# sortmerna/sortmerna

Hardware: AMD Instinct MI355X
Metric: reads/sec (150 bp vs smr_v4.3_default_db-sized DB) (higher is better)
Workload: dtype u8/i32

## Files before the change

### sortmerna_amd/csrc/smr_engine.hip

```cpp
#include <hip/hip_runtime.h>

#include <algorithm>
#include <mutex>
#include <cstdio>
#include <cstdlib>
#include <cstring>
#include <string>
#include <vector>

#include "smr_kernels.hpp"
#include "smr_idcov.hpp"
#include "smr_ibuild.hpp"
#include "smr_pgbuild.hpp"
#include "smr_hostmem.hpp"

using namespace smr;

namespace {

struct DevIndex {
  bool used = false;
  Lookup* lookup = nullptr; uint32_t* trie = nullptr; uint32_t* pos_off = nullptr; uint2* pos_arr = nullptr;
  uint32_t* pg = nullptr; uint32_t* root3 = nullptr; uint32_t* lkc = nullptr;
  uint8_t* ref_seq = nullptr; uint64_t* ref_off = nullptr;
// ... 8 lines not shown

#define SMR_MAX_BATCHES 16
enum { KP_KEYS = 0, KP_SPLIT, KP_BINS, KP_PG0, KP_PG1, KP_FINISH, KP_CAND, KP_CHAIN, KP_BEGINS, KP_TRACE, KP_WALK, KP_SW16, KP_WNEXT, KP_IDCOV, KP_COUNT };
static const char* const KP_NAME[KP_COUNT] = {"k_seed_keys", "k_seed_split", "k_seed_bins", "k_seed_pg<0>", "k_seed_pg<1>", "k_seed_finish", "k_cand", "k_chain", "k_begins", "k_trace",
                                              "k_walk", "k_sw16", "k_wnext", "k_idcov"};

struct Batch {
  bool used = false;
  uint32_t n = 0, max_len = 0, slots = 1;
  uint32_t min_ge[7] = {~0u, ~0u, ~0u, ~0u, ~0u, ~0u, ~0u};
  uint64_t gen = 0;
  bool min_ge_known = false;
  uint32_t* d_words = nullptr; uint64_t* d_rec_off = nullptr; uint32_t* d_len = nullptr;
  RState* d_saved = nullptr; RState* d_work = nullptr; RWork* d_rw = nullptr;
  uint8_t* d_marks = nullptr;
  AlignRec* d_saved_aln = nullptr; AlignRec* d_work_aln = nullptr;
  unsigned long long* d_ctr = nullptr;
  uint32_t* d_cigar = nullptr; uint64_t cigar_words = 0;
  uint32_t* d_idcov = nullptr; size_t cap_idcov = 0; bool idcov_ran = false;
  std::vector<uint32_t> h_idcov;
  std::vector<RState> h_state; std::vector<AlignRec> h_aln; std::vector<uint32_t> h_cigar;
  std::vector<uint32_t> h_idx, h_map;
  uint32_t last_num_alignments = 1;
  unsigned long long redo_seen = 0, win_seen = 0;
  bool fetched = false;
  size_t cap_words = 0, cap_reads = 0, cap_aln = 0;
};

struct SharedSet { SeedTup* srt = nullptr; uint16_t* wbin = nullptr; uint32_t* cbase = nullptr; uint32_t* sn = nullptr; uint32_t maxwin = 0; bool built = false; };
struct SharedSort {
  SharedSet set[2][3];
  const void* batch = nullptr; uint64_t gen = 0; uint32_t lnwin = 0, skip[3] = {0, 0, 0}, n = 0, max_len = 0;
  uint64_t cap[3] = {0, 0, 0};
  bool usable = false;
  uint32_t* abits = nullptr; size_t abits_words = 0;
};

struct smr_ctx {
  int device = 0;
  hipStream_t stream = nullptr;
  std::string err;
  std::mutex err_m, sel_m;
  int n_cu = 256;
  DevIndex idx[64];
  Batch bt[SMR_MAX_BATCHES];
  Batch* b = &bt[0];
  uint32_t* d_pool = nullptr; uint64_t pool_words = 0;
  uint64_t n_pool_grown = 0;
  uint32_t pool_inline = 0;
  uint32_t hcap = 4;
  int seed_exact = 0;
  uint32_t cand_bloom = 128;
  uint32_t hot_min = getenv("SMR_SEED_DEDUP") ? (uint32_t)std::max(0, atoi(getenv("SMR_SEED_DEDUP"))) : 1024u;
  int seed_shared = getenv("SMR_SEED_SHARED") ? atoi(getenv("SMR_SEED_SHARED")) : 1;
  uint16_t* d_sw_scr = nullptr; uint32_t sw_scr_stride = 0; size_t sw_scr_words = 0;
  int last_seed_slot = -1;
  SharedSort* shared = nullptr;
  uint64_t n_seed_shared = 0, n_seed_shared_builds = 0;
  uint32_t ccap = PG_CAND_CAP0;
  uint32_t pg_grid = getenv("SMR_PG_GRID") ? (uint32_t)atoi(getenv("SMR_PG_GRID")) : 262144u;
  int pg_swz = getenv("SMR_PG_SWZ") ? atoi(getenv("SMR_PG_SWZ")) : 0;
  SeedBufs sb = {};
  uint64_t sb_slots = 0; uint32_t sb_nk = 0;
  uint32_t chain_blocks = 0;
  unsigned long long* d_tuples = nullptr; uint32_t chain_scap = 512;
  uint32_t keys_need = 0;
  bool chain_ext = false;
  uint32_t* d_stab = nullptr; unsigned long long* d_tuples2 = nullptr;
  size_t chain_lds_attr = 0, begins_lds_attr = 0, split_lds_attr = 0, bins_lds_attr = 0;
  uint32_t* d_fidx = nullptr; RState* d_fstate = nullptr; AlignRec* d_faln = nullptr; size_t fetch_cap_r = 0, fetch_cap_a = 0;
  uint32_t* d_fidcov = nullptr; size_t fetch_cap_i = 0;
  int sw_mode = getenv("SMR_SW_PACKED") ? atoi(getenv("SMR_SW_PACKED")) : 2;
  unsigned long long* d_keys = nullptr; uint32_t keys_cap = 0;
  unsigned long long* d_pairs = nullptr; uint32_t* d_lis = nullptr; uint32_t pairs_cap = 0;
  uint2* d_hits = nullptr; uint32_t hits_cap = 0;
  uint8_t* d_rdq = nullptr; size_t rdq_cap = 0;
  int handover = getenv("SMR_HANDOVER") ? atoi(getenv("SMR_HANDOVER")) : 1;
  uint2* d_mrec = nullptr; uint32_t* d_mpool = nullptr; size_t mrec_cap = 0, mpool_words = 0;
  int walk_split = getenv("SMR_WALK_SPLIT") ? atoi(getenv("SMR_WALK_SPLIT")) : 1;
  uint32_t walk_rounds = getenv("SMR_WALK_ROUNDS") ? (uint32_t)std::max(1, std::min(32, atoi(getenv("SMR_WALK_ROUNDS")))) : 8u;
  uint32_t walk_k = getenv("SMR_WALK_K") ? (uint32_t)std::max(1, std::min((int)WK_MAX, atoi(getenv("SMR_WALK_K")))) : 4u;
  int walk_gather = getenv("SMR_WALK_GATHER") ? atoi(getenv("SMR_WALK_GATHER")) : 1;
  uint32_t walk_assume = getenv("SMR_WALK_ASSUME") ? (uint32_t)atoi(getenv("SMR_WALK_ASSUME")) : 3u;
  uint2* d_wlist[2] = {nullptr, nullptr}; WState* d_wstate[2] = {nullptr, nullptr}; WTask* d_wtask[2] = {nullptr, nullptr}; uint2* d_wres[2] = {nullptr, nullptr};
  uint32_t* d_wtidx = nullptr; uint32_t* d_wslow = nullptr; unsigned long long* d_wctr = nullptr; size_t walk_cap = 0; uint32_t walk_kcap = 0, walk_rcap = 0;
  size_t walk_lds_attr = 0, pg_lds_attr = 0, search_lds_attr = 0;
  uint64_t sw16_launches[8] = {};
  bool walk_rounds_fixed = getenv("SMR_WALK_ROUNDS") != nullptr;
  uint32_t walk_need[3] = {0, 0, 0};
  unsigned long long* d_wstat = nullptr; uint32_t wstat_n = 0; int wstat_pass[8] = {}; uint32_t wstat_rm[8] = {};
  int* d_bound = nullptr; size_t bound_cap = 0;
  uint32_t* d_tasks = nullptr; uint64_t tasks_cap = 0;
  uint8_t* d_trflags = nullptr; uint64_t trflags_bytes = 0;
  int* d_trrows = nullptr; uint64_t trrows_ints = 0;
  std::vector<EvMark> events; std::vector<hipEvent_t> ev_pool;
  double kp_ms[KP_COUNT] = {}; uint64_t kp_l[KP_COUNT] = {};
  hipStream_t upload_stream = nullptr;
  unsigned long long* d_ctr_snap = nullptr;
};
struct KpSave { double ms[KP_COUNT]; uint64_t l[KP_COUNT]; };

#define SEED_REDO_CAP 16384u

namespace {

#define HIPCHK(ctx, call)                                                                        \
  do {                                                                                           \
    hipError_t e_ = (call);                                                                      \
    if (e_ != hipSuccess) {                                                                      \
      std::lock_guard<std::mutex> l_((ctx)->err_m);                                              \
      (ctx)->err = std::string(#call) + ": " + hipGetErrorString(e_);                            \
      return SMR_ERR_DEVICE;                                                                     \
    }                                                                                            \
  } while (0)

void set_err(smr_ctx* c, const std::string& msg) { std::lock_guard<std::mutex> l_(c->err_m); c->err = msg; }

template <class T> int dev_alloc(smr_ctx* c, T** p, size_t count) {
  if (*p) { (void)hipFree(*p); *p = nullptr; }
  if (count == 0) count = 1;
  HIPCHK(c, hipMalloc((void**)p, count * sizeof(T)));
  return SMR_OK;
}
template <class T> void dev_free(T** p) { if (*p) { (void)hipFree(*p); *p = nullptr; } }


const char* scheme_unsupported(int mismatch, int score_N, int gap_open, int gap_ext);
DParams make_dparams(const smr_ctx* c, const DevIndex& di, const smr_params* p) {
  DParams P;
  memset(&P, 0, sizeof P);
  P.lnwin = di.lnwin; P.partialwin = di.lnwin / 2;
  if (p->skiplengths[0] == 0 || p->skiplengths[1] == 0 || p->skiplengths[2] == 0) {
    P.skip[0] = di.lnwin; P.skip[1] = di.lnwin / 2; P.skip[2] = 3;
  } else { P.skip[0] = p->skiplengths[0]; P.skip[1] = p->skiplengths[1]; P.skip[2] = p->skiplengths[2]; }
  P.num_seeds = p->num_seeds; P.min_lis = p->min_lis; P.edges = p->edges; P.is_as_percent = p->is_as_percent;
  P.match = p->match; P.mismatch = p->mismatch; P.score_N = p->score_N; P.gap_open = p->gap_open; P.gap_ext = p->gap_ext;
  P.minimal_score = p->minimal_score; P.num_alignments = p->num_alignments;
  P.is_best = p->is_best; P.is_full_search = p->is_full_search; P.is_forward = p->is_forward; P.is_reverse = p->is_reverse;
  P.minoccur = p->minoccur; P.index_num = p->index_num; P.part = p->part; P.is_last_index_part = p->is_last_index_part;
  P.slots = c->b->slots;
  P.sw_mode = scheme_unsupported(p->mismatch, p->score_N, p->gap_open, p->gap_ext) ? -1 : c->sw_mode;
  P.sw_scratch = c->d_sw_scr; P.sw_scratch_stride = c->sw_scr_stride;
  return P;
}

const char* scheme_unsupported(int mismatch, int score_N, int gap_open, int gap_ext) {
  const int mm = std::max(-mismatch, -std::min(score_N, 0));
  if (2 * gap_open < mm || 2 * gap_ext < mm) return "scoring scheme outside the supported range (2*gap_open and 2*gap_ext must be >= |mismatch|)";
  if (score_N > 0) return "scoring scheme outside the supported range (score_N must be <= 0: the kernels pad sequences with N)";
  if (gap_open <= gap_ext) return "scoring scheme outside the supported range (gap_open must be greater than gap_ext: the reference's 16-bit kernel ends its lazy-F loop early otherwise, ssw.c:496-507)";
  return nullptr;
}

int check_params(smr_ctx* c, const smr_params* p, bool sw = true) {
  if (!p) { set_err(c, "null params"); return SMR_ERR_ARG; }
  if (p->index_num >= 64) { set_err(c, "index_num must be < 64"); return SMR_ERR_ARG; }
  if ((uint64_t)p->minoccur >= 0x3FFFFFFFull) { set_err(c, "minoccur must be < 2^30 - 1"); return SMR_ERR_ARG; }
  if (p->num_seeds < 1 || p->gap_open < 0 || p->gap_ext < 0 || p->match <= 0 || p->mismatch > 0) { set_err(c, "bad scoring/seed options"); return SMR_ERR_ARG; }
  if (p->match > 127 || p->mismatch < -127 || p->score_N > 127 || p->score_N < -127 || p->gap_open > 255 || p->gap_ext > 255) { set_err(c, "scores must fit int8 / gaps uint8 like the reference's"); return SMR_ERR_ARG; }
  if (sw && (p->edges < 1 || p->edges > 10)) { set_err(c, "edges must be 1..10 (nucleotides or percent), like the reference's --edges"); return SMR_ERR_ARG; }
  if (p->num_alignments > 0 && p->num_alignments > c->b->slots) { set_err(c, "num_alignments exceeds max_alignments_per_read given to smr_reads_upload"); return SMR_ERR_ARG; }
  return SMR_OK;
}

DIndex dindex(const DevIndex& d) {
  DIndex x; x.lookup = d.lookup; x.trie = d.trie; x.pg = d.pg; x.lkc = d.lkc; x.root3 = reinterpret_cast<const uint2*>(d.root3); x.pos_off = d.pos_off; x.pos_arr = d.pos_arr; x.ref_seq = d.ref_seq; x.ref_off = d.ref_off;
// ... 852 lines not shown
```

### sortmerna_amd/csrc/smr_engine_chain.hpp

```cpp

uint32_t chain_edges(const DParams& P, uint32_t len) { return P.is_as_percent ? (uint32_t)((P.edges / 100.0) * len) + 1 : (uint32_t)std::max(P.edges, 0); }
void chain_lds(const smr_ctx* c, const DParams& P, uint32_t& ml, uint32_t& rf, uint32_t& rq, size_t& bytes) {
  const uint32_t mq_len = std::min<uint32_t>(c->b->max_len, SW_X4_MAX_ROWS);
  ml = (c->b->max_len + 15) & ~15u;
  rf = (c->b->max_len + 2 * chain_edges(P, c->b->max_len) + 16 + 15) & ~15u;
  rq = std::min(rf, (mq_len + 2 * chain_edges(P, mq_len) + 16 + 15) & ~15u);
  bytes = 5 * (size_t)std::min<uint32_t>(ml, SW_X4_MAX_ROWS) + (size_t)9 * rq + (size_t)CH_KEYS_LDS * 8 + (size_t)std::max<uint32_t>(4u * CH_PAIRS_LDS, 2u * c->chain_scap) * 4 +
          (size_t)CH_HITS_LDS * 8 + (size_t)(CH_HITS_LDS + 8) * 4 + (size_t)c->chain_scap * 4;
}
void chain_lds(const smr_ctx* c, const DParams& P, uint32_t& ml, uint32_t& rf, size_t& bytes) { uint32_t rq; chain_lds(c, P, ml, rf, rq, bytes); }
int ensure_bound(smr_ctx* c, uint32_t blocks, uint32_t rf) {
  if (c->b->max_len <= SW_X4_MAX_ROWS) return SMR_OK;
  const size_t need = (size_t)blocks * 2 * rf, need_rd = (size_t)blocks * ((c->b->max_len + 15) & ~15u);
  if (c->bound_cap < need) { int rc = dev_alloc(c, &c->d_bound, need); if (rc) return rc; c->bound_cap = need; }
  if (c->rdq_cap < need_rd) { int rc = dev_alloc(c, &c->d_rdq, need_rd); if (rc) return rc; c->rdq_cap = need_rd; }
  return SMR_OK;
}

__global__ void k_wstat(const unsigned long long* __restrict__ wctr, unsigned long long* __restrict__ out, uint32_t rounds) {
  if (threadIdx.x < 32) out[threadIdx.x] = threadIdx.x < rounds ? wctr[(size_t)threadIdx.x * WC_STRIDE + WC_NLIST] : 0ull;
}
int adapt_walk_rounds(smr_ctx* c) {
  if (c->walk_rounds_fixed || !c->wstat_n || !c->d_wstat) return SMR_OK;
  unsigned long long h[8 * 32];
  HIPCHK(c, hipMemcpyAsync(h, c->d_wstat, (size_t)c->wstat_n * 32 * 8, hipMemcpyDeviceToHost, c->stream));
  HIPCHK(c, hipStreamSynchronize(c->stream));
  const unsigned long long few = (unsigned long long)c->n_cu * 8ull;
  uint32_t need[3] = {0, 0, 0};
  for (uint32_t e = 0; e < c->wstat_n; e++) {
    uint32_t want = 2;
    for (uint32_t r = 0; r < c->wstat_rm[e]; r++) if (h[e * 32 + r] > few) want = r + 2 + (r + 1 == c->wstat_rm[e] ? 2u : 0u);
    need[c->wstat_pass[e]] = std::max(need[c->wstat_pass[e]], want);
  }
  for (int p = 0; p < 3; p++) if (need[p]) {
    const uint32_t prev = c->walk_need[p] ? c->walk_need[p] : c->walk_rounds;
    c->walk_need[p] = std::min(c->walk_rounds, need[p] >= prev ? need[p] : prev - std::max(1u, (prev - need[p]) / 2u));
  }
  c->wstat_n = 0;
  return SMR_OK;
}

int launch_chain(smr_ctx* c, const DevIndex& di, const DParams& P, int pass, int is_last_strand) {
  uint32_t ml, rf, rq; size_t lds;
  chain_lds(c, P, ml, rf, rq, lds);
  HIPCHK(c, hipMemsetAsync(&c->b->d_ctr[C_WORK_NEXT], 0, 8, c->stream));
  if (lds > 64 * 1024 && lds > c->chain_lds_attr) {
    HIPCHK(c, hipFuncSetAttribute((const void*)k_chain<false, false>, hipFuncAttributeMaxDynamicSharedMemorySize, (int)lds));
    HIPCHK(c, hipFuncSetAttribute((const void*)k_chain<true, false>, hipFuncAttributeMaxDynamicSharedMemorySize, (int)lds));
    HIPCHK(c, hipFuncSetAttribute((const void*)k_chain<false, true>, hipFuncAttributeMaxDynamicSharedMemorySize, (int)lds));
    HIPCHK(c, hipFuncSetAttribute((const void*)k_chain<true, true>, hipFuncAttributeMaxDynamicSharedMemorySize, (int)lds));
    HIPCHK(c, hipFuncSetAttribute((const void*)k_chain<false, false, true>, hipFuncAttributeMaxDynamicSharedMemorySize, (int)lds));
    HIPCHK(c, hipFuncSetAttribute((const void*)k_chain<true, false, true>, hipFuncAttributeMaxDynamicSharedMemorySize, (int)lds));
    HIPCHK(c, hipFuncSetAttribute((const void*)k_chain<false, true, true>, hipFuncAttributeMaxDynamicSharedMemorySize, (int)lds));
    HIPCHK(c, hipFuncSetAttribute((const void*)k_chain<true, true, true>, hipFuncAttributeMaxDynamicSharedMemorySize, (int)lds));
    c->chain_lds_attr = lds;
  }
  uint32_t blocks = std::min<uint32_t>(c->chain_blocks, std::max(c->b->n, 1u));
  { int rc = ensure_bound(c, c->chain_blocks, rf); if (rc) return rc; }
  int* const gb = c->b->max_len > SW_X4_MAX_ROWS ? c->d_bound : nullptr;
  uint8_t* const grd = c->b->max_len > SW_X4_MAX_ROWS ? c->d_rdq : nullptr;
  if (c->handover) {
    const size_t want_w = (size_t)((c->b->n + CAND_BLOCK - 1u) / CAND_BLOCK) * CAND_BLOCK * CAND_REC_WORDS;
    if (c->mrec_cap < c->b->n) { int rc = dev_alloc(c, &c->d_mrec, (size_t)c->b->n); if (rc) return rc; c->mrec_cap = c->b->n; }
    if (c->mpool_words < want_w) { int rc = dev_alloc(c, &c->d_mpool, want_w); if (rc) return rc; c->mpool_words = want_w; }
  }
  uint2* const mrec = c->handover ? c->d_mrec : nullptr;
  const uint32_t wmq = std::min<uint32_t>(c->b->max_len, WK_MAX_ROWS), wml = (wmq + 15) & ~15u;
  const bool split = c->walk_split && mrec && P.sw_mode >= 1 && sw_pk_fits((int)wmq, (int)rq, P.match, P.mismatch, P.score_N, P.gap_open);
  const uint32_t RMX = c->walk_rounds, WK = c->walk_k;
  const uint32_t RM = (!c->walk_rounds_fixed && c->walk_need[pass]) ? std::min(RMX, c->walk_need[pass]) : RMX;
  if (split) {
    const size_t n = c->b->n;
    if (c->walk_cap < n || c->walk_kcap < WK) {
      for (int q = 0; q < 2; q++) {
        int rc;
        if ((rc = dev_alloc(c, &c->d_wlist[q], n)) || (rc = dev_alloc(c, &c->d_wstate[q], n)) || (rc = dev_alloc(c, &c->d_wtask[q], n * WK)) || (rc = dev_alloc(c, &c->d_wres[q], n * WK))) return rc;
      }
      int rc;
      if ((rc = dev_alloc(c, &c->d_wtidx, 2 * n * WK)) || (rc = dev_alloc(c, &c->d_wslow, n))) return rc;
      c->walk_cap = n; c->walk_kcap = WK;
    }
    if (c->walk_rcap < RMX) { int rc = dev_alloc(c, &c->d_wctr, (size_t)(RMX + 2) * WC_STRIDE); if (rc) return rc; if ((rc = dev_alloc(c, &c->d_wstat, (size_t)8 * 32))) return rc; c->walk_rcap = RMX; }
    HIPCHK(c, hipMemsetAsync(c->d_wctr, 0, (size_t)(RMX + 2) * WC_STRIDE * 8, c->stream));
    const size_t lds_w = (size_t)wml + rq;
    if (lds_w > 64 * 1024 && lds_w > c->walk_lds_attr) { HIPCHK(c, hipFuncSetAttribute((const void*)k_walk<true>, hipFuncAttributeMaxDynamicSharedMemorySize, (int)lds_w)); c->walk_lds_attr = lds_w; }
  }
  const size_t n_tix = (size_t)c->walk_cap * c->walk_kcap;
  unsigned long long* const n_slow = split ? c->d_wctr + (size_t)(RMX + 1) * WC_STRIDE : nullptr;
  ev_mark(c, KP_CAND);
  hipLaunchKernelGGL(k_cand, dim3((c->b->n + CAND_BLOCK - 1u) / CAND_BLOCK), dim3(256), CAND_LDS_BYTES(c->cand_bloom, c->handover), c->stream, dreads(c), dindex(di), P, pass, is_last_strand, c->b->d_work, c->b->d_rw, (const uint32_t*)c->d_pool, c->b->d_marks, c->cand_bloom,
                     mrec, c->d_mpool, c->mpool_words);
  if (split) {
    ev_mark(c, KP_WNEXT);
    hipLaunchKernelGGL(k_wlist, dim3((c->b->n + 1023u) / 1024u), dim3(1024), 0, c->stream, dreads(c), c->b->d_marks, (const uint2*)mrec, (uint32_t)WK_MAX_ROWS, c->d_wlist[0], c->d_wslow, c->d_wctr, n_slow, getenv("SMR_WALK_DEBUG") ? n_slow + 8 : (unsigned long long*)nullptr, (P.num_seeds >= 2 && c->walk_gather) ? 1 : 0);
    const int swr = wmq <= 104 ? 13 : wmq <= 152 ? 19 : wmq <= 208 ? 26 : 32;
    const uint32_t walk_blocks = (uint32_t)c->n_cu * 4u * SMR_WALK_WAVES_PER_SIMD, sw_blocks = (uint32_t)c->n_cu * 4u * (uint32_t)SW16_WAVES(swr);
    for (uint32_t rnd = 0; rnd < RM; rnd++) {
      const int cur = (int)(rnd & 1u), prv = cur ^ 1;
      unsigned long long* const wc = c->d_wctr + (size_t)rnd * WC_STRIDE;
      const bool fin = rnd + 1 == RM;
      ev_mark(c, KP_WALK);
#define WALK_ARGS dreads(c), dindex(di), P, pass, is_last_strand, c->b->d_work, c->b->d_work_aln, c->b->d_rw, c->b->d_ctr, (const uint2*)mrec, (const uint32_t*)c->d_mpool, (const uint32_t*)c->d_pool, (const uint2*)c->d_wlist[cur], \
                  (const WState*)c->d_wstate[prv], (const WTask*)c->d_wtask[prv], (const uint2*)c->d_wres[prv], c->d_wstate[cur], c->d_wtask[cur], c->d_wtidx, c->d_wtidx + n_tix, wc, WK, (unsigned long long)n_tix, (int)rnd, wml, rq, c->walk_assume
      if (fin) hipLaunchKernelGGL(k_walk<true>, dim3(walk_blocks * 3u / SMR_WALK_WAVES_PER_SIMD), dim3(64), (size_t)wml + rq, c->stream, WALK_ARGS);
      else {
        hipLaunchKernelGGL(k_walk<false>, dim3(walk_blocks), dim3(64), 0, c->stream, WALK_ARGS);
        ev_mark(c, KP_SW16);
#define SW16_ARGS dreads(c), dindex(di), P, (const WTask*)c->d_wtask[cur], (const uint32_t*)c->d_wtidx, (const uint32_t*)(c->d_wtidx + n_tix), (const unsigned long long*)wc, c->d_wres[cur]
        if (swr == 13) hipLaunchKernelGGL(k_sw16<13>, dim3(sw_blocks), dim3(64), 0, c->stream, SW16_ARGS);
        else if (swr == 19) hipLaunchKernelGGL(k_sw16<19>, dim3(sw_blocks), dim3(64), 0, c->stream, SW16_ARGS);
        else if (swr == 26) hipLaunchKernelGGL(k_sw16<26>, dim3(sw_blocks), dim3(64), 0, c->stream, SW16_ARGS);
        else hipLaunchKernelGGL(k_sw16<32>, dim3(sw_blocks), dim3(64), 0, c->stream, SW16_ARGS);
#undef SW16_ARGS
        c->sw16_launches[swr == 13 ? 0 : swr == 19 ? 1 : swr == 26 ? 2 : 3]++;
        ev_mark(c, KP_WNEXT);
        hipLaunchKernelGGL(k_wnext, dim3((uint32_t)c->n_cu * 2u), dim3(1024), 0, c->stream, P, is_last_strand, c->b->d_work, c->b->d_rw, c->b->d_ctr, (const uint2*)c->d_wlist[cur], (const WState*)c->d_wstate[cur],
                           (const uint2*)c->d_wres[cur], c->d_wlist[prv], (const unsigned long long*)wc, wc + WC_STRIDE, WK, (unsigned long long)n_tix, (int)rnd);
      }
#undef WALK_ARGS
    }
    if (!c->walk_rounds_fixed && c->wstat_n < 8) {
      hipLaunchKernelGGL(k_wstat, dim3(1), dim3(32), 0, c->stream, (const unsigned long long*)c->d_wctr, c->d_wstat + (size_t)c->wstat_n * 32, RM);
      c->wstat_pass[c->wstat_n] = pass; c->wstat_rm[c->wstat_n] = RM; c->wstat_n++;
    }
    if (getenv("SMR_WALK_DEBUG")) {
      std::vector<unsigned long long> h((size_t)(RMX + 2) * WC_STRIDE);
      HIPCHK(c, hipMemcpyAsync(h.data(), c->d_wctr, h.size() * 8, hipMemcpyDeviceToHost, c->stream));
      HIPCHK(c, hipStreamSynchronize(c->stream));
      { const unsigned long long* q = &h[(size_t)(RMX + 1) * WC_STRIDE];
        fprintf(stderr, "libsmr_hip: walk rounds (pass %d): slow %llu (positions <= 64 / 128 / 256 / 512 / more / > 64 hits: %llu %llu %llu %llu %llu %llu);", pass, q[0], q[8], q[9], q[10], q[11], q[12], q[13]); }
      for (uint32_t rnd = 0; rnd < RM; rnd++) fprintf(stderr, " %llu/%llu+%llu", h[(size_t)rnd * WC_STRIDE + WC_NLIST], h[(size_t)rnd * WC_STRIDE + WC_NTASK], h[(size_t)rnd * WC_STRIDE + WC_NTASK2]);
      fprintf(stderr, "\n");
    }
  }
  ev_mark(c, KP_CHAIN);
#define CHAIN_ARGS(stab, t2) dreads(c), dindex(di), P, pass, is_last_strand, c->b->d_work, c->b->d_work_aln, c->b->d_rw, c->d_pool, c->b->d_ctr, c->d_tuples, c->d_keys, c->d_pairs, \
                             c->d_lis, c->d_hits, c->keys_cap, c->pairs_cap, c->hits_cap, ml, rf, c->chain_scap, stab, t2, rq, gb, grd, c->b->d_marks, (const uint2*)mrec, (const uint32_t*)c->d_mpool, \
                             (const uint32_t*)(split ? c->d_wslow : nullptr), (const unsigned long long*)n_slow
  const bool striped = P.sw_mode < 0;
  if (striped) {
    if (gb) hipLaunchKernelGGL((k_chain<false, true, true>), dim3(blocks), dim3(64), lds, c->stream, CHAIN_ARGS(c->chain_ext ? c->d_stab : nullptr, c->chain_ext ? c->d_tuples2 : nullptr));
    else hipLaunchKernelGGL((k_chain<false, false, true>), dim3(blocks), dim3(64), lds, c->stream, CHAIN_ARGS(c->chain_ext ? c->d_stab : nullptr, c->chain_ext ? c->d_tuples2 : nullptr));
  } else
  if (gb) hipLaunchKernelGGL((k_chain<false, true>), dim3(blocks), dim3(64), lds, c->stream, CHAIN_ARGS(c->chain_ext ? c->d_stab : nullptr, c->chain_ext ? c->d_tuples2 : nullptr));
  else hipLaunchKernelGGL((k_chain<false, false>), dim3(blocks), dim3(64), lds, c->stream, CHAIN_ARGS(c->chain_ext ? c->d_stab : nullptr, c->chain_ext ? c->d_tuples2 : nullptr));
  if (c->chain_ext) {
    HIPCHK(c, hipMemsetAsync(&c->b->d_ctr[C_WORK_NEXT], 0, 8, c->stream));
    if (striped) {
      if (gb) hipLaunchKernelGGL((k_chain<true, true, true>), dim3(blocks), dim3(64), lds, c->stream, CHAIN_ARGS(c->d_stab, c->d_tuples2));
      else hipLaunchKernelGGL((k_chain<true, false, true>), dim3(blocks), dim3(64), lds, c->stream, CHAIN_ARGS(c->d_stab, c->d_tuples2));
    } else
    if (gb) hipLaunchKernelGGL((k_chain<true, true>), dim3(blocks), dim3(64), lds, c->stream, CHAIN_ARGS(c->d_stab, c->d_tuples2));
    else hipLaunchKernelGGL((k_chain<true, false>), dim3(blocks), dim3(64), lds, c->stream, CHAIN_ARGS(c->d_stab, c->d_tuples2));
  }
#undef CHAIN_ARGS
  ev_stop(c);
  HIPCHK(c, hipGetLastError());
  return SMR_OK;
}

void fold_shards(std::vector<unsigned long long>& h) {
  for (int s = 0; s < C_NSHARD; s++)
    for (int k = 0; k < C_SHARD_W; k++) {
      if (k < C_SHARD_X) h[C_WINDOWS + k] += h[C_SHARDS + C_SHARD_W * s + k];
      else if (k < C_SHARD_X + C_SHARD_NX) h[C_TUP_F + k - C_SHARD_X] += h[C_SHARDS + C_SHARD_W * s + k];
      h[C_SHARDS + C_SHARD_W * s + k] = 0;
    }
  unsigned long long mx = 0;
  for (int s = 0; s < C_NSHARD; s++) mx = std::max(mx, h[C_PCUR + s * C_PCUR_STRIDE]);
  h[C_POOL_CURSOR] = mx;
}

int read_ctr(smr_ctx* c, std::vector<unsigned long long>& h) {
  h.resize(C_TOTAL);
  HIPCHK(c, hipMemcpyAsync(h.data(), c->b->d_ctr, C_TOTAL * 8, hipMemcpyDeviceToHost, c->stream));
  HIPCHK(c, hipStreamSynchronize(c->stream));
  fold_shards(h);
  return SMR_OK;
}
```

### sortmerna_amd/csrc/smr_walk.hpp

```cpp
#pragma once

namespace smr {

#define WK_MAX 15u
__host__ __device__ __forceinline__ uint32_t walk_tasks_per_read(uint32_t nlist, unsigned long long cap, uint32_t k0, int round) {
  if (round == 0) return k0;
  const unsigned long long q = nlist ? cap / nlist : (unsigned long long)WK_MAX;
  return (uint32_t)(q < k0 ? k0 : (q > WK_MAX ? WK_MAX : q));
}
#define WK_MAX_ROWS 256u
#define WK_MAX_POS 128u
#ifndef WK_CLAIM
#define WK_CLAIM 24u
#endif
enum { WC_NLIST = 0, WC_CLAIM = 16, WC_NTASK = 32, WC_NTASK2 = 48, WC_STRIDE = 64 };

struct WTask {
  uint32_t r, max_ref;
  uint64_t rf_start;
  uint32_t ars, head;
  uint16_t aq, m, nref;
  uint16_t flags;
};
struct WState {
  uint32_t k, it, ms_lo, ms_hi, begin_ref, begin_read;
  int32_t best;
  uint32_t bits;
  uint32_t cells;
};
#define WS_NK(bits) (((bits) >> 8) & 15u)

__global__ void __launch_bounds__(1024) k_wlist(DReads rd, uint8_t* __restrict__ marks, const uint2* __restrict__ mrec, uint32_t max_rows, uint2* __restrict__ list0,
                                                uint32_t* __restrict__ slow, unsigned long long* __restrict__ wc0, unsigned long long* __restrict__ n_slow, unsigned long long* census, int gather) {
  const uint32_t i = blockIdx.x * blockDim.x + threadIdx.x;
  const bool mk = i < rd.n && marks[i] == 1;
  const bool fast = mk && mrec && (mrec[i].x != NONE || (mrec[i].y - 1u < WK_MAX_POS && gather)) && rd.len[i] <= max_rows;
  const uint32_t o = block_append(&wc0[WC_NLIST], fast);
  if (fast) { list0[o] = make_uint2(i, NONE); marks[i] = 0; }
  const uint32_t o2 = block_append(n_slow, mk && !fast);
  if (mk && !fast) slow[o2] = i;
  if (census) {
    const uint32_t np = (mk && !fast && mrec) ? mrec[i].y : 0u;
    const bool s = mk && !fast;
    const int cls = !s ? -1 : np == 0xFFFFFFFFu ? 5 : np <= 64u ? 0 : np <= 128u ? 1 : np <= 256u ? 2 : np <= 512u ? 3 : 4;
    for (int q = 0; q < 6; q++) { const unsigned long long m = __ballot(cls == q); if (m && (threadIdx.x & 63u) == 0) atomicAdd(&census[q], (unsigned long long)__popcll(m)); }
  }
}

__device__ __forceinline__ int dpp_quad_ror1(int v) { return __builtin_amdgcn_update_dpp(v, v, 0x93 , 0xF, 0xF, false); }
template <int U> __device__ __forceinline__ int dpp_quad_bcast(int v) { return __builtin_amdgcn_update_dpp(v, v, U * 0x55 , 0xF, 0xF, false); }
__device__ __forceinline__ unsigned long long quad_max_u64(unsigned long long v) {
  for (int d = 2; d > 0; d >>= 1) { const unsigned long long o = __shfl_xor(v, d, 64); v = o > v ? o : v; }
  return v;
}

struct __attribute__((aligned(4))) Sw16W3 { uint32_t a, b, c; };
struct __attribute__((aligned(4))) Sw16W2 { uint32_t a, b; };
template <int R, bool HASN, bool KEYS>
__device__ __forceinline__ SwRes sw_quad16(const uint32_t* __restrict__ rec, uint32_t len, uint32_t reversed, int m, int aq, const uint8_t* __restrict__ ref, int n,
                                           int match, int mismatch, int scoreN, int go, int ge, int dir) {
  const int gl = lane_id() & 3;
  const pk16 GE = pk_splat(ge), GO = pk_splat(go), ZERO = pk_splat(0);
  const uint32_t TN = (((uint32_t)(scoreN + go)) & 0xFFFFu) * 0x00010001u;
  uint32_t tlo[R], thi[R];
  pk16 Y[R], E[R];
  uint32_t key[KEYS ? R : 1];
  pk16 hmax = ZERO;
  const uint32_t t_mm = ((uint32_t)(mismatch + go) & 0xFFu) * 0x01010101u, t_x = ((uint32_t)(mismatch + go) ^ (uint32_t)(match + go)) & 0xFFu,
                 t_n = ((uint32_t)(scoreN + go) & 0xFFu) * 0x01010101u;
  const uint32_t cw = (len + 15u) >> 4, cwm = max(cw, 1u) - 1u, awm = max((len + 31u) >> 5, 1u) - 1u;
  const int sgn = reversed ? -dir : dir;
  uint32_t cwd[2][3], awd[2][2];
  int pa[2], cw0[2], aw0[2];
#pragma unroll
  for (int hf = 0; hf < 2; hf++) {
    const int row0 = (gl + 4 * hf) * R, nv = max(1, min(R, m - row0));
    const int k0 = aq + dir * row0;
    pa[hf] = reversed ? (int)len - 1 - k0 : k0;
    const int pmin = max(0, min(pa[hf], pa[hf] + sgn * (nv - 1)));
    cw0[hf] = (int)min((uint32_t)pmin >> 4, cwm); aw0[hf] = (int)min((uint32_t)pmin >> 5, awm);
    const Sw16W3 c3 = *reinterpret_cast<const Sw16W3*>(rec + cw0[hf]);
    const Sw16W2 a2 = *reinterpret_cast<const Sw16W2*>(rec + cw + aw0[hf]);
    cwd[hf][0] = c3.a; cwd[hf][1] = c3.b; cwd[hf][2] = c3.c; awd[hf][0] = a2.a; awd[hf][1] = a2.b;
  }
#pragma unroll
  for (int j = 0; j < R; j++) {
    uint32_t t2[2];
#pragma unroll
    for (int hf = 0; hf < 2; hf++) {
      const int row = (gl + 4 * hf) * R + j;
      uint32_t t = 0;
      if (row < m) {
        const int ph = pa[hf] + sgn * j;
        const int wi = (ph >> 4) - cw0[hf], ai = (ph >> 5) - aw0[hf];
        const uint32_t wd = wi == 0 ? cwd[hf][0] : wi == 1 ? cwd[hf][1] : cwd[hf][2];
        const uint32_t ad = ai == 0 ? awd[hf][0] : awd[hf][1];
        uint32_t c = (wd >> ((ph & 15) * 2)) & 3u;
        if (reversed) c = 3u - c;
        if ((ad >> (ph & 31)) & 1u) c = 4u;
        t = c == 4u ? t_n : t_mm ^ (t_x << (8u * c));
      }
      t2[hf] = t;
    }
    tlo[j] = t2[0]; thi[j] = t2[1];
    Y[j] = pk_splat(-go); E[j] = ZERO; if (KEYS) key[j] = 0;
  }
  int steps = m > 0 ? n + (m + R - 1) / R - 1 : 0;
  for (int d = 32; d > 0; d >>= 1) steps = max(steps, __shfl_xor(steps, d, 64));
#ifdef SMR_SW16_NOSTEPS
  steps = min(steps, 4);
#endif
  uint32_t lastY = pk_bits(pk_splat(-go)), lastF = 0, selcur = PK_SEL_NONE * 0x00010001u;
  pk16 diag0 = pk_splat(-go);
// ... 56 lines not shown
  unsigned long long k64 = bestH > 0 ? (((unsigned long long)bestH << 42) | ((unsigned long long)(0x1FFFFF - bestcol) << 21) |
                                        (unsigned long long)(0x1FFFFF - bestrow)) : 0ull;
  k64 = quad_max_u64(k64);
  SwRes rr;
  if (k64 == 0) { rr.score = 0; rr.end_ref = -1; rr.end_read = m - 1; return rr; }
  rr.score = (int)(k64 >> 42);
  rr.end_ref = 0x1FFFFF - (int)((k64 >> 21) & 0x1FFFFF);
  rr.end_read = 0x1FFFFF - (int)(k64 & 0x1FFFFF);
  return rr;
}

__device__ __forceinline__ uint2 wres_pack(const SwRes& s) { return make_uint2((uint32_t)s.score, s.end_ref < -1 ? 0xFFFFFFFFu : ((uint32_t)(s.end_ref + 1) << 16) | ((uint32_t)s.end_read & 0xFFFFu)); }
__device__ __forceinline__ SwRes wres_unpack(const uint2 v) {
  SwRes s; s.score = (int)v.x;
  if (v.y == 0xFFFFFFFFu) { s.end_ref = -2; s.end_read = 0; }
  else { s.end_ref = (int)(v.y >> 16) - 1; s.end_read = (int)(v.y & 0xFFFFu); }
  return s;
}

#ifndef SW16_WAVES
#define SW16_WAVES(R) ((R) <= 13 ? 4 : (R) <= 19 ? 3 : 2)
#endif
template <int R>
__global__ void __launch_bounds__(64, SW16_WAVES(R)) k_sw16(DReads rd, DIndex ix, DParams P, const WTask* __restrict__ tk, const uint32_t* __restrict__ tidx1,
                                                           const uint32_t* __restrict__ tidx2, const unsigned long long* __restrict__ wc, uint2* __restrict__ res) {
  const int lane = lane_id(), g = lane >> 2, gl = lane & 3;
  const uint32_t ntA = (uint32_t)wc[WC_NTASK], ntB = (uint32_t)wc[WC_NTASK2];
  const uint32_t npassA = (ntA + 15u) / 16u, npass = npassA + (ntB + 15u) / 16u;
  auto slot_of = [&](uint32_t p) -> uint32_t {
    const bool keys = p < npassA;
    const uint32_t ti = (keys ? p : p - npassA) * 16u + (uint32_t)g;
    return (p < npass && ti < (keys ? ntA : ntB)) ? (keys ? tidx1 : tidx2)[ti] : NONE;
  };
  uint32_t slot_next = slot_of(blockIdx.x);
  for (uint32_t p = blockIdx.x; p < npass; p += gridDim.x) {
    const bool keys = p < npassA;
    const uint32_t ti = (keys ? p : p - npassA) * 16u + (uint32_t)g;
    const uint32_t* const tidx = keys ? tidx1 : tidx2;
    const uint32_t slot = slot_next;
    const bool have = slot != NONE;
    int m = 0, n = 0, aq = 0, dir = 1;
    uint32_t len = 0, reversed = 0;
    const uint32_t* rec = rd.words;
    const uint8_t* ref = ix.ref_seq;
    if (have) {
      const WTask t = tk[slot];
      m = t.m; n = t.nref; aq = t.aq; reversed = t.flags & 1u; dir = (t.flags & 2u) ? -1 : 1;
      len = rd.len[t.r]; rec = rd.words + rd.rec_off[t.r];
      ref = ix.ref_seq + t.rf_start;
    }
    slot_next = slot_of(p + gridDim.x);
    int nn = n;
    for (int d = 32; d > 0; d >>= 1) nn = max(nn, __shfl_xor(nn, d, 64));
    bool hn = false;
    if (ix.ref_any_n) {
      const int nm = max(n, 1) - 1;
      for (int q0 = gl; q0 < nn; q0 += 32) {
        uint8_t b[8];
#pragma unroll
        for (int i = 0; i < 8; i++) b[i] = ref[dir * min(q0 + 4 * i, nm)];
#pragma unroll
        for (int i = 0; i < 8; i++) hn |= (q0 + 4 * i < n) && b[i] == 4;
      }
    }
    SwRes s;
    const bool hasn = __any(hn);
#define SW16_ARGS rec, len, reversed, m, aq, ref, n, P.match, P.mismatch, P.score_N, P.gap_open, P.gap_ext, dir
    if (keys) { if (hasn) s = sw_quad16<R, true, true>(SW16_ARGS); else s = sw_quad16<R, false, true>(SW16_ARGS); }
    else { if (hasn) s = sw_quad16<R, true, false>(SW16_ARGS); else s = sw_quad16<R, false, false>(SW16_ARGS); }
#undef SW16_ARGS
    if (have && gl == 0) res[tidx[ti]] = wres_pack(s);
  }
}

#ifndef SMR_WALK_WAVES_PER_SIMD
#define SMR_WALK_WAVES_PER_SIMD 5
#endif
template <bool FINAL>
__global__ void __launch_bounds__(64, FINAL ? 3 : SMR_WALK_WAVES_PER_SIMD)
k_walk(DReads rd, DIndex ix, DParams P, int pass, int is_last_strand, RState* __restrict__ work, AlignRec* __restrict__ work_aln, RWork* __restrict__ rw,
       unsigned long long* __restrict__ ctr, const uint2* __restrict__ mrec, const uint32_t* __restrict__ mpool, const uint32_t* __restrict__ pool,
       const uint2* __restrict__ list, const WState* __restrict__ ws_prev, const WTask* __restrict__ tk_prev, const uint2* __restrict__ res_prev,
       WState* __restrict__ ws_cur, WTask* __restrict__ tk_cur, uint32_t* __restrict__ tidx, uint32_t* __restrict__ tidx2, unsigned long long* __restrict__ wc,
       uint32_t K0, unsigned long long task_cap, int round, uint32_t lds_ml, uint32_t lds_rf, uint32_t assume_min) {
  SMR_DYN_LDS(unsigned char, lds_raw);
  __shared__ unsigned long long l_pairs[WK_MAX_POS];
  __shared__ uint2 l_cand[64];
  __shared__ unsigned long long l_cref[64];
  __shared__ uint32_t l_clen[64];
  __shared__ uint32_t l_hkey[256], l_hcnt[256];
  __shared__ unsigned long long l_stage[WK_MAX_POS];
  __shared__ WTask s_ctk[WK_MAX];
  __shared__ uint2 s_cres[WK_MAX];
  __shared__ uint32_t s_tix[WK_CLAIM * WK_MAX];
  __shared__ uint32_t s_next, s_tbase;
  const int lane = lane_id();
  const uint32_t nlist = (uint32_t)wc[WC_NLIST];
  const uint32_t K = walk_tasks_per_read(nlist, task_cap, K0, round);
  const uint32_t Kp = round > 0 ? walk_tasks_per_read((uint32_t)(wc - WC_STRIDE)[WC_NLIST], task_cap, K0, round - 1) : K0;
  unsigned long long n_fwd = 0, n_cells = 0, n_spec = 0, n_spec_used = 0, n_newhit = 0;
#ifdef SMR_WALK_PHASES
  unsigned long long wph[7] = {0, 0, 0, 0, 0, 0, 0}, wlast = clock64();
#define WPH(i) { const unsigned long long tn_ = clock64(); wph[i] += tn_ - wlast; wlast = tn_; }
#else
#define WPH(i)
#endif
  const uint32_t claim = max(1u, min(WK_CLAIM, nlist / (gridDim.x * 4u)));
  for (;;) {
    __syncthreads();
    if (lane == 0) s_next = (uint32_t)atomicAdd(&wc[WC_CLAIM], (unsigned long long)claim);
    __syncthreads();
    const uint32_t chunk_base = s_next;
    if (chunk_base >= nlist) break;
    const uint32_t chunk_n = min(claim, nlist - chunk_base);
    uint32_t ntix = 0, ntix2 = 0;
    uint32_t c_r = 0, c_prev = NONE, c_len = 0;
    uint2 c_mr = make_uint2(NONE, 0u);
    if ((uint32_t)lane < chunk_n) { const uint2 le = list[chunk_base + lane]; c_r = le.x; c_prev = le.y; c_mr = mrec[c_r]; c_len = rd.len[c_r]; }
    for (uint32_t ci = 0; ci < chunk_n; ci++) {
      const uint32_t e = chunk_base + ci;
      const uint32_t r = (uint32_t)__builtin_amdgcn_readlane((int)c_r, (int)ci), prev = (uint32_t)__builtin_amdgcn_readlane((int)c_prev, (int)ci);
      const uint32_t len = (uint32_t)__builtin_amdgcn_readlane((int)c_len, (int)ci);
      const uint2 mr = make_uint2((uint32_t)__builtin_amdgcn_readlane((int)c_mr.x, (int)ci), (uint32_t)__builtin_amdgcn_readlane((int)c_mr.y, (int)ci));
      RWork w = rw[r];
      RState st = work[r];
      const uint32_t* rec = FINAL ? rd.words + rd.rec_off[r] : nullptr;
      WState ps; ps.bits = 0;
      if (prev != NONE) ps = ws_prev[prev];
      uint32_t live_bits = 0;
      if (w.strand_active && w.search && w.pass_n == (uint32_t)pass && mr.y - 1u < WK_MAX_POS) {
        WPH(0)
        const uint32_t npos = mr.y;
        uint32_t seq[2] = {0, 0}, pos[2] = {0, 0}, win[2] = {0, 0};
        const bool valid[2] = {(uint32_t)lane < npos, (uint32_t)lane + 64u < npos};
        __syncthreads();
        if (mr.x != NONE) {
          const uint32_t* rp = mpool + mr.x;
          if (valid[0]) { seq[0] = rp[lane]; pos[0] = rp[npos + lane]; win[0] = rp[2u * npos + lane]; }
        } else {
          uint32_t* const g_hp = (uint32_t*)l_stage;
          uint32_t* const g_lo = g_hp + 65, * const g_wn = g_lo + 64;
          const uint32_t nh = w.hit_total;
          uint32_t lo = 0, ln = 0;
          if ((uint32_t)lane < nh) {
            const uint32_t h = (uint32_t)lane, c0 = w.blk_cnt[0], c1 = w.blk_cnt[1];
            const uint32_t at = h < c0 ? w.blk_off[0] + 2 * h : h - c0 < c1 ? w.blk_off[1] + 2 * (h - c0) : w.blk_off[2] + 2 * (h - c0 - c1);
            const uint32_t id = pool[at];
            g_wn[lane] = pool[at + 1];
            lo = id + 1u; ln = ix.pos_arr[id].x;
          }
          uint32_t tot;
          const uint32_t ex = wave_excl_scan_u32(ln, tot);
          if ((uint32_t)lane < nh) { g_hp[lane] = ex; g_lo[lane] = lo; }
          if (lane == 0) g_hp[nh] = tot;
          __syncthreads();
#pragma unroll
          for (int q = 0; q < 2; q++) if (valid[q]) {
            const uint32_t p = (uint32_t)lane + 64u * q;
            uint32_t h = 0;
            for (uint32_t step = 32; step > 0; step >>= 1) { const uint32_t t = h + step; if (t < nh && g_hp[t] <= p) h = t; }
            const uint2 pa = ix.pos_arr[g_lo[h] + (p - g_hp[h])];
            seq[q] = pa.y; pos[q] = pa.x; win[q] = g_wn[h];
          }
          __syncthreads();
        }
#pragma unroll
        for (int q = 0; q < 4; q++) { l_hkey[lane + 64 * q] = 0xFFFFFFFFu; l_hcnt[lane + 64 * q] = 0; }
        __syncthreads();
        uint32_t slot[2] = {0, 0};
#pragma unroll
        for (int q = 0; q < 2; q++) if (valid[q]) {
          uint32_t sl = (seq[q] * 0x9E3779B1u) >> 24;
          for (;;) { const uint32_t o = atomicCAS(&l_hkey[sl], 0xFFFFFFFFu, seq[q]); if (o == 0xFFFFFFFFu || o == seq[q]) break; sl = (sl + 1u) & 255u; }
          atomicAdd(&l_hcnt[sl], 1u);
          slot[q] = sl;
        }
        __threadfence_block();
        __syncthreads();
        const bool mem0 = valid[0] && (int)l_hcnt[slot[0]] >= P.num_seeds, mem1 = valid[1] && (int)l_hcnt[slot[1]] >= P.num_seeds;
        const unsigned long long mm0 = __ballot(mem0), mm1 = __ballot(mem1);
        const uint32_t tot0 = (uint32_t)__popcll(mm0), total = tot0 + (uint32_t)__popcll(mm1);
        const unsigned long long ltm = (1ull << lane) - 1ull;
        if (mem0) l_stage[__popcll(mm0 & ltm)] = ((unsigned long long)slot[0] << 48) | ((unsigned long long)pos[0] << 16) | (unsigned long long)(win[0] & 0xFFFFu);
        if (mem1) l_stage[tot0 + (uint32_t)__popcll(mm1 & ltm)] = ((unsigned long long)slot[1] << 48) | ((unsigned long long)pos[1] << 16) | (unsigned long long)(win[1] & 0xFFFFu);
        __syncthreads();
        if (total > 64) wave_sort_u64(l_stage, total);
        else if (total > 1) {
          unsigned long long key = (uint32_t)lane < total ? l_stage[lane] : ~0ull;
          uint32_t np2 = 2; while (np2 < total) np2 <<= 1;
          for (uint32_t kk = 2; kk <= np2; kk <<= 1)
            for (uint32_t j = kk >> 1; j > 0; j >>= 1) {
              const unsigned long long o = __shfl_xor(key, (int)j, 64);
              const bool want_min = (((uint32_t)lane & j) == 0) == (((uint32_t)lane & kk) == 0);
              if (want_min ? o < key : key < o) key = o;
            }
          if ((uint32_t)lane < total) l_stage[lane] = key;
        }
        __syncthreads();
        unsigned long long key2[2]; bool head[2]; uint32_t sl2[2];
#pragma unroll
        for (int q = 0; q < 2; q++) {
          const uint32_t i = (uint32_t)lane + 64u * q;
          key2[q] = i < total ? l_stage[i] : ~0ull;
          sl2[q] = (uint32_t)(key2[q] >> 48) & 255u;
          head[q] = i < total && (i == 0 || sl2[q] != ((uint32_t)(l_stage[i - (i ? 1u : 0u)] >> 48) & 255u));
        }
        const unsigned long long h0 = __ballot(head[0]), h1 = __ballot(head[1]);
        const uint32_t ncand = (uint32_t)__popcll(h0) + (uint32_t)__popcll(h1);
        uint32_t count[2], hseq[2];
        {
          const unsigned long long ab0 = lane < 63 ? h0 >> (lane + 1) : 0ull, ab1 = lane < 63 ? h1 >> (lane + 1) : 0ull;
          const uint32_t e0 = ab0 ? (uint32_t)lane + (uint32_t)__ffsll((long long)ab0) : h1 ? 63u + (uint32_t)__ffsll((long long)h1) : total;
          const uint32_t e1 = ab1 ? 64u + (uint32_t)lane + (uint32_t)__ffsll((long long)ab1) : total;
          count[0] = e0 - (uint32_t)lane; count[1] = e1 - (64u + (uint32_t)lane);
          hseq[0] = head[0] ? l_hkey[sl2[0]] : 0u; hseq[1] = head[1] ? l_hkey[sl2[1]] : 0u;
        }
        const unsigned long long my0 = ((unsigned long long)(0xFFFFFFFFu - count[0]) << 32) | hseq[0], my1 = ((unsigned long long)(0xFFFFFFFFu - count[1]) << 32) | hseq[1];
        uint32_t rank0 = 0, rank1 = 0;
        for (unsigned long long mq = h0; mq; mq &= mq - 1) {
          const int c = __ffsll((long long)mq) - 1;
          const unsigned long long key_c = ((unsigned long long)(0xFFFFFFFFu - (uint32_t)__builtin_amdgcn_readlane((int)count[0], c)) << 32) | (uint32_t)__builtin_amdgcn_readlane((int)hseq[0], c);
          rank0 += key_c < my0 ? 1u : 0u; rank1 += key_c < my1 ? 1u : 0u;
        }
        for (unsigned long long mq = h1; mq; mq &= mq - 1) {
          const int c = __ffsll((long long)mq) - 1;
          const unsigned long long key_c = ((unsigned long long)(0xFFFFFFFFu - (uint32_t)__builtin_amdgcn_readlane((int)count[1], c)) << 32) | (uint32_t)__builtin_amdgcn_readlane((int)hseq[1], c);
          rank0 += key_c < my0 ? 1u : 0u; rank1 += key_c < my1 ? 1u : 0u;
        }
        __syncthreads();
#pragma unroll
        for (int q = 0; q < 2; q++) {
          const uint32_t i = (uint32_t)lane + 64u * q;
          if (i < total) l_pairs[i] = ((key2[q] >> 16) << 32) | (key2[q] & 0xFFFFull);
          if (head[q]) {
            const uint32_t rk = q ? rank1 : rank0;
            const uint64_t r0_ = ix.ref_off[hseq[q]], r1_ = ix.ref_off[hseq[q] + 1];
            l_cand[rk] = make_uint2(hseq[q], count[q] | (i << 8));
            l_cref[rk] = r0_; l_clen[rk] = (uint32_t)(r1_ - r0_);
          }
        }
        const uint32_t n_prev = prev != NONE ? WS_NK(ps.bits) : 0u;
        if ((uint32_t)lane < n_prev) { s_ctk[lane] = tk_prev[(size_t)prev * Kp + lane]; s_cres[lane] = res_prev[(size_t)prev * Kp + lane]; }
        __syncthreads();
        WPH(1)

        struct Walk { uint32_t k, it, ms_lo, ms_hi, begin_ref, begin_read; int is_aligned, best, go_on, started, pending_pop; };
        const uint64_t rlen = len;
        auto load_candidate = [&](Walk& wk) -> int {
          if (wk.k >= ncand || !wk.go_on) return 0;
          const uint32_t cy = l_cand[wk.k].y;
          const uint32_t max_occur = cy & 0xFFu;
          if (max_occur < (uint32_t)P.num_seeds) return 0;
          if (wk.is_aligned && P.min_lis > 0 && wk.k > 0 && max_occur < (l_cand[wk.k - 1].y & 0xFFu)) {
            --wk.best;
            if (wk.best < 1) return 0;
          }
          const unsigned long long p0 = l_pairs[cy >> 8];
          wk.it = 0; wk.ms_lo = 0; wk.ms_hi = 0;
          wk.begin_ref = (uint32_t)(p0 >> 32); wk.begin_read = (uint32_t)p0;
          wk.pending_pop = 0;
          return 1;
        };
        auto next_task = [&](Walk& wk, SwTask& tk) -> bool {
          const uint2 ce = l_cand[wk.k];
          const unsigned long long* pairs = l_pairs + (ce.y >> 8);
          const uint32_t np = ce.y & 0xFFu;
          while (wk.it != np && wk.go_on) {
            if (!wk.pending_pop) {
              wk.pending_pop = 1;
              const uint64_t end_ref_max = (uint64_t)wk.begin_ref + len - wk.begin_read - P.lnwin + 1;
              int push = 0;
              for (;;) {
                const uint32_t pi = wk.it + (uint32_t)lane;
                const bool okp = pi < np && (uint64_t)(uint32_t)(pairs[min(pi, np - 1)] >> 32) <= end_ref_max;
                const unsigned long long pm = __ballot(okp);
                const uint32_t pc = pm == ~0ull ? 64u : (uint32_t)__ffsll((long long)~pm) - 1u;
                if (pc) { wk.it += pc; wk.ms_hi = wk.it; push = 1; }
                if (pc < 64u) break;
              }
              int skip_to_pop = 0;
              if (!push && wk.is_aligned) skip_to_pop = 1;
              else wk.is_aligned = 0;
              if (!skip_to_pop && (wk.ms_hi - wk.ms_lo) >= (uint32_t)P.num_seeds) {
                uint32_t lis0;
                const uint32_t nw = wk.ms_hi - wk.ms_lo;
                uint32_t* const lisb = (uint32_t*)l_stage;
                const uint32_t nl = nw <= 64 ? wave_lis_first(pairs + wk.ms_lo, nw, lis0) : serial_lis_first(pairs + wk.ms_lo, nw, lisb, lisb + WK_MAX_POS, lis0);
                if (nl >= (uint32_t)P.min_lis) {
                  const unsigned long long pl = pairs[wk.ms_lo + lis0];
                  const uint32_t lcs_ref_start = (uint32_t)(pl >> 32), lcs_que_start = (uint32_t)pl;
                  const uint64_t reflen = l_clen[wk.k];
                  uint64_t hd = 0, tail = 0, align_ref_start = 0, align_que_start = 0, align_length = 0;
                  uint32_t edges;
                  if (P.is_as_percent) edges = (uint32_t)((P.edges / 100.0) * (double)rlen);
                  else edges = (uint32_t)P.edges;
                  if (lcs_ref_start < lcs_que_start) {
                    align_ref_start = 0; align_que_start = lcs_que_start - lcs_ref_start; hd = 0;
                    if (reflen < rlen) {
                      tail = 0;
                      if (align_que_start > (rlen - reflen)) align_length = reflen - (align_que_start - (rlen - reflen));
                      else align_length = reflen;
                    } else {
                      tail = reflen - align_ref_start - rlen;
                      if (tail > (uint64_t)(uint32_t)(edges - 1)) tail = edges;
                      align_length = rlen + hd + tail - align_que_start;
                    }
                  } else {
                    align_ref_start = lcs_ref_start - lcs_que_start; align_que_start = 0;
                    if (align_ref_start > (uint64_t)(uint32_t)(edges - 1)) hd = edges;
                    if (align_ref_start + rlen > reflen) { tail = 0; align_length = reflen - align_ref_start - hd; }
                    else {
                      tail = reflen - align_ref_start - rlen;
                      if (tail > (uint64_t)(uint32_t)(edges - 1)) tail = edges;
                      align_length = rlen + hd + tail;
                    }
                  }
                  tk.max_ref = ce.x; tk.align_ref_start = align_ref_start; tk.head = hd; tk.align_que_start = align_que_start;
                  tk.m = (int)(align_length - hd - tail); tk.nref = (int)align_length;
                  tk.rf_start = l_cref[wk.k] + align_ref_start - hd;
                  return true;
                }
              }
            }
            wk.pending_pop = 0;
            if (wk.ms_hi > wk.ms_lo) wk.ms_lo++;
// ... 267 lines not shown
```

Baseline: 54.41 million.

## Prefetch next read's walk state and rows one iteration ahead in k_walk

The walk kernel now loads the next read's RWork, RState, previous WState, match-pool rows and previous task/result rows into per-lane registers during the current iteration, spreading the struct loads across lanes (one word per lane) and broadcasting them with readlane. This is meant to hide the global memory latency of the serial per-read loads inside the chunk loop. It also adds an optional env knob that fixes the claim size. Costs are extra registers and some wasted loads for reads that end up skipped.

Measured after the change: 54.92 million, median of 6. About the same (+0.9%).

```diff
diff --git a/sortmerna_amd/csrc/smr_engine.hip b/sortmerna_amd/csrc/smr_engine.hip
--- a/sortmerna_amd/csrc/smr_engine.hip
+++ b/sortmerna_amd/csrc/smr_engine.hip
@@ -114,6 +114,7 @@
   uint32_t walk_k = getenv("SMR_WALK_K") ? (uint32_t)std::max(1, std::min((int)WK_MAX, atoi(getenv("SMR_WALK_K")))) : 4u;
   int walk_gather = getenv("SMR_WALK_GATHER") ? atoi(getenv("SMR_WALK_GATHER")) : 1;
   uint32_t walk_assume = getenv("SMR_WALK_ASSUME") ? (uint32_t)atoi(getenv("SMR_WALK_ASSUME")) : 3u;
+  uint32_t walk_claim = getenv("SMR_WALK_CLAIM") ? (uint32_t)std::max(0, atoi(getenv("SMR_WALK_CLAIM"))) : 0u;
   uint2* d_wlist[2] = {nullptr, nullptr}; WState* d_wstate[2] = {nullptr, nullptr}; WTask* d_wtask[2] = {nullptr, nullptr}; uint2* d_wres[2] = {nullptr, nullptr};
   uint32_t* d_wtidx = nullptr; uint32_t* d_wslow = nullptr; unsigned long long* d_wctr = nullptr; size_t walk_cap = 0; uint32_t walk_kcap = 0, walk_rcap = 0;
   size_t walk_lds_attr = 0, pg_lds_attr = 0, search_lds_attr = 0;
diff --git a/sortmerna_amd/csrc/smr_engine_chain.hpp b/sortmerna_amd/csrc/smr_engine_chain.hpp
--- a/sortmerna_amd/csrc/smr_engine_chain.hpp
+++ b/sortmerna_amd/csrc/smr_engine_chain.hpp
@@ -101,7 +101,7 @@
       const bool fin = rnd + 1 == RM;
       ev_mark(c, KP_WALK);
 #define WALK_ARGS dreads(c), dindex(di), P, pass, is_last_strand, c->b->d_work, c->b->d_work_aln, c->b->d_rw, c->b->d_ctr, (const uint2*)mrec, (const uint32_t*)c->d_mpool, (const uint32_t*)c->d_pool, (const uint2*)c->d_wlist[cur], \
-                  (const WState*)c->d_wstate[prv], (const WTask*)c->d_wtask[prv], (const uint2*)c->d_wres[prv], c->d_wstate[cur], c->d_wtask[cur], c->d_wtidx, c->d_wtidx + n_tix, wc, WK, (unsigned long long)n_tix, (int)rnd, wml, rq, c->walk_assume
+                  (const WState*)c->d_wstate[prv], (const WTask*)c->d_wtask[prv], (const uint2*)c->d_wres[prv], c->d_wstate[cur], c->d_wtask[cur], c->d_wtidx, c->d_wtidx + n_tix, wc, WK, (unsigned long long)n_tix, (int)rnd, wml, rq, c->walk_assume, c->walk_claim
       if (fin) hipLaunchKernelGGL(k_walk<true>, dim3(walk_blocks * 3u / SMR_WALK_WAVES_PER_SIMD), dim3(64), (size_t)wml + rq, c->stream, WALK_ARGS);
       else {
         hipLaunchKernelGGL(k_walk<false>, dim3(walk_blocks), dim3(64), 0, c->stream, WALK_ARGS);
diff --git a/sortmerna_amd/csrc/smr_walk.hpp b/sortmerna_amd/csrc/smr_walk.hpp
--- a/sortmerna_amd/csrc/smr_walk.hpp
+++ b/sortmerna_amd/csrc/smr_walk.hpp
@@ -29,6 +29,10 @@
   uint32_t cells;
 };
 #define WS_NK(bits) (((bits) >> 8) & 15u)
+typedef uint32_t __attribute__((may_alias)) walk_word;
+enum { WPF_RW = sizeof(RWork) / 4, WPF_ST = sizeof(RState) / 4, WPF_WS = sizeof(WState) / 4 };
+static_assert(sizeof(RWork) % 4 == 0 && sizeof(RState) % 4 == 0 && sizeof(WState) % 4 == 0 && WPF_RW + WPF_ST + WPF_WS <= 64, "k_walk: one word per lane");
+static_assert(sizeof(WTask) == 32 && WK_MAX * sizeof(WTask) / 4 <= 128 && WK_MAX * 2 <= 64, "k_walk: a read's task rows are two words per lane, its result rows one");
 
 __global__ void __launch_bounds__(1024) k_wlist(DReads rd, uint8_t* __restrict__ marks, const uint2* __restrict__ mrec, uint32_t max_rows, uint2* __restrict__ list0,
                                                 uint32_t* __restrict__ slow, unsigned long long* __restrict__ wc0, unsigned long long* __restrict__ n_slow, unsigned long long* census, int gather) {
@@ -251,7 +255,7 @@
        unsigned long long* __restrict__ ctr, const uint2* __restrict__ mrec, const uint32_t* __restrict__ mpool, const uint32_t* __restrict__ pool,
        const uint2* __restrict__ list, const WState* __restrict__ ws_prev, const WTask* __restrict__ tk_prev, const uint2* __restrict__ res_prev,
        WState* __restrict__ ws_cur, WTask* __restrict__ tk_cur, uint32_t* __restrict__ tidx, uint32_t* __restrict__ tidx2, unsigned long long* __restrict__ wc,
-       uint32_t K0, unsigned long long task_cap, int round, uint32_t lds_ml, uint32_t lds_rf, uint32_t assume_min) {
+       uint32_t K0, unsigned long long task_cap, int round, uint32_t lds_ml, uint32_t lds_rf, uint32_t assume_min, uint32_t claim_fix) {
   SMR_DYN_LDS(unsigned char, lds_raw);
   __shared__ unsigned long long l_pairs[WK_MAX_POS];
   __shared__ uint2 l_cand[64];
@@ -274,7 +278,8 @@
 #else
 #define WPH(i)
 #endif
-  const uint32_t claim = max(1u, min(WK_CLAIM, nlist / (gridDim.x * 4u)));
+  const uint32_t claim = claim_fix ? min(WK_CLAIM, claim_fix) : max(1u, min(WK_CLAIM, nlist / (gridDim.x * 4u)));
+  uint32_t pf_u = 0, pf_row[3] = {0, 0, 0}, pf_tk[2] = {0, 0}, pf_rs = 0;
   for (;;) {
     __syncthreads();
     if (lane == 0) s_next = (uint32_t)atomicAdd(&wc[WC_CLAIM], (unsigned long long)claim);
@@ -285,17 +290,45 @@
     uint32_t ntix = 0, ntix2 = 0;
     uint32_t c_r = 0, c_prev = NONE, c_len = 0;
     uint2 c_mr = make_uint2(NONE, 0u);
-    if ((uint32_t)lane < chunk_n) { const uint2 le = list[chunk_base + lane]; c_r = le.x; c_prev = le.y; c_mr = mrec[c_r]; c_len = rd.len[c_r]; }
+    uint64_t c_ro = 0;
+    if ((uint32_t)lane < chunk_n) { const uint2 le = list[chunk_base + lane]; c_r = le.x; c_prev = le.y; c_mr = mrec[c_r]; c_len = rd.len[c_r]; if (FINAL) c_ro = rd.rec_off[c_r]; }
+    auto prefetch = [&](uint32_t ci) {
+      const uint32_t r = (uint32_t)__builtin_amdgcn_readlane((int)c_r, (int)ci), prev = (uint32_t)__builtin_amdgcn_readlane((int)c_prev, (int)ci);
+      const uint32_t mx = (uint32_t)__builtin_amdgcn_readlane((int)c_mr.x, (int)ci), np = (uint32_t)__builtin_amdgcn_readlane((int)c_mr.y, (int)ci);
+      const uint32_t l = min((uint32_t)lane, prev != NONE ? (uint32_t)(WPF_RW + WPF_ST + WPF_WS) - 1u : (uint32_t)(WPF_RW + WPF_ST) - 1u);
+      const walk_word* const src = l < (uint32_t)WPF_RW ? (const walk_word*)(rw + r) + l : l < (uint32_t)(WPF_RW + WPF_ST) ? (const walk_word*)(work + r) + (l - WPF_RW)
+                                                                                                                  : (const walk_word*)(ws_prev + prev) + (l - (WPF_RW + WPF_ST));
+      pf_u = *src;
+      if (mx != NONE && np - 1u < WK_MAX_POS) {
+        const uint32_t* const rp = mpool + mx;
+        const uint32_t li = min((uint32_t)lane, np - 1u);
+        pf_row[0] = rp[li]; pf_row[1] = rp[np + li]; pf_row[2] = rp[2u * np + li];
+      }
+      if (prev != NONE) {
+        const walk_word* const tp = (const walk_word*)(tk_prev + (size_t)prev * Kp);
+        const walk_word* const sp = (const walk_word*)(res_prev + (size_t)prev * Kp);
+        const uint32_t tw = Kp * (uint32_t)(sizeof(WTask) / 4) - 1u;
+        pf_tk[0] = tp[min((uint32_t)lane, tw)]; pf_tk[1] = tp[min((uint32_t)lane + 64u, tw)]; pf_rs = sp[min((uint32_t)lane, 2u * Kp - 1u)];
+      }
+    };
+    prefetch(0);
     for (uint32_t ci = 0; ci < chunk_n; ci++) {
       const uint32_t e = chunk_base + ci;
       const uint32_t r = (uint32_t)__builtin_amdgcn_readlane((int)c_r, (int)ci), prev = (uint32_t)__builtin_amdgcn_readlane((int)c_prev, (int)ci);
       const uint32_t len = (uint32_t)__builtin_amdgcn_readlane((int)c_len, (int)ci);
       const uint2 mr = make_uint2((uint32_t)__builtin_amdgcn_readlane((int)c_mr.x, (int)ci), (uint32_t)__builtin_amdgcn_readlane((int)c_mr.y, (int)ci));
-      RWork w = rw[r];
-      RState st = work[r];
-      const uint32_t* rec = FINAL ? rd.words + rd.rec_off[r] : nullptr;
-      WState ps; ps.bits = 0;
-      if (prev != NONE) ps = ws_prev[prev];
+      RWork w; RState st; WState ps;
+      {
+        uint32_t uw[WPF_RW + WPF_ST + WPF_WS];
+#pragma unroll
+        for (int q = 0; q < WPF_RW + WPF_ST + WPF_WS; q++) uw[q] = (uint32_t)__builtin_amdgcn_readlane((int)pf_u, q);
+        __builtin_memcpy(&w, uw, sizeof(RWork)); __builtin_memcpy(&st, uw + WPF_RW, sizeof(RState)); __builtin_memcpy(&ps, uw + WPF_RW + WPF_ST, sizeof(WState));
+        if (prev == NONE) ps.bits = 0;
+      }
+      const uint32_t row_s = pf_row[0], row_p = pf_row[1], row_w = pf_row[2], tk_w0 = pf_tk[0], tk_w1 = pf_tk[1], rs_w = pf_rs;
+      if (ci + 1u < chunk_n) prefetch(ci + 1u);
+      const uint32_t* rec = nullptr;
+      if (FINAL) rec = rd.words + (((uint64_t)(uint32_t)__builtin_amdgcn_readlane((int)(uint32_t)(c_ro >> 32), (int)ci) << 32) | (uint32_t)__builtin_amdgcn_readlane((int)(uint32_t)c_ro, (int)ci));
       uint32_t live_bits = 0;
       if (w.strand_active && w.search && w.pass_n == (uint32_t)pass && mr.y - 1u < WK_MAX_POS) {
         WPH(0)
@@ -303,9 +336,14 @@
         uint32_t seq[2] = {0, 0}, pos[2] = {0, 0}, win[2] = {0, 0};
         const bool valid[2] = {(uint32_t)lane < npos, (uint32_t)lane + 64u < npos};
         __syncthreads();
+        if (prev != NONE) {
+          const uint32_t tw = Kp * (uint32_t)(sizeof(WTask) / 4);
+          if ((uint32_t)lane < tw) ((walk_word*)s_ctk)[lane] = tk_w0;
+          if ((uint32_t)lane + 64u < tw) ((walk_word*)s_ctk)[lane + 64] = tk_w1;
+          if ((uint32_t)lane < 2u * Kp) ((walk_word*)s_cres)[lane] = rs_w;
+        }
         if (mr.x != NONE) {
-          const uint32_t* rp = mpool + mr.x;
-          if (valid[0]) { seq[0] = rp[lane]; pos[0] = rp[npos + lane]; win[0] = rp[2u * npos + lane]; }
+          if (valid[0]) { seq[0] = row_s; pos[0] = row_p; win[0] = row_w; }
         } else {
           uint32_t* const g_hp = (uint32_t*)l_stage;
           uint32_t* const g_lo = g_hp + 65, * const g_wn = g_lo + 64;
@@ -409,7 +447,6 @@
           }
         }
         const uint32_t n_prev = prev != NONE ? WS_NK(ps.bits) : 0u;
-        if ((uint32_t)lane < n_prev) { s_ctk[lane] = tk_prev[(size_t)prev * Kp + lane]; s_cres[lane] = res_prev[(size_t)prev * Kp + lane]; }
         __syncthreads();
         WPH(1)
 
```
